# blairstar/NaturalDiffusion

Measured on AMD Instinct MI355X. Metric: images/sec at 15-step Natural Inference (CIFAR10 32x32, NCSN++), 3-stream throughput, higher is better.
Workload: dtype bf16; 1 GPU; CIFAR10 NI 15-step step_15_weight_173.npz B=512/GPU NCSN++ 61.8M bf16, ni_step fp64 history; nfe=15, batch_per_gpu=512, streams=3

## Files before the change

### include/natinf_ncsnpp.h

```cpp
#ifndef NATINF_NCSNPP_H
#define NATINF_NCSNPP_H

#include <stdint.h>
#include "natinf.h"

#ifdef __cplusplus
extern "C" {
#endif

typedef struct natinf_ncsnpp* natinf_ncsnpp_t;

#define NATINF_NCSNPP_KEEP_ACTIVATIONS 1
#define NATINF_NCSNPP_DDPM 2

int64_t natinf_ncsnpp_param_count(void);
int64_t natinf_ncsnpp_packed_bytes(void);
int64_t natinf_ncsnpp_handle_param_count(natinf_ncsnpp_t h);
int64_t natinf_ncsnpp_handle_packed_bytes(natinf_ncsnpp_t h);
int64_t natinf_ncsnpp_workspace_bytes(natinf_ncsnpp_t h, int max_batch);

int natinf_ncsnpp_create(natinf_ncsnpp_t* out, int flags);
int natinf_ncsnpp_destroy(natinf_ncsnpp_t h);

int natinf_ncsnpp_describe(natinf_ncsnpp_t h, char* buf, int cap);
// ... 22 lines not shown
int natinf_debug_conv_gn_fin(float* fin_scale, float* fin_shift, const float* gamma, const float* beta, int channels_per_group, float mul);
int natinf_debug_conv_gn(int res, int B, int N, int cin, int c1, const void* x, const float* scale, const float* shift, const void* w_packed, void* w_frag,
                         const void* a1, const float* bias_n, const void* resid, float out_scale, void* out, float* gn_part, int iters,
                         natinf_stream_t stream);
#define NATINF_ATTN_BLOCK_OFF_WQKV 0
#define NATINF_ATTN_BLOCK_OFF_W3 393216
#define NATINF_ATTN_BLOCK_OFF_FOLD_WQK 524288
#define NATINF_ATTN_BLOCK_OFF_FOLD_WVO 786432
#define NATINF_ATTN_BLOCK_OFF_FOLD_CQ 1048576
#define NATINF_ATTN_BLOCK_OFF_FOLD_BO 1049600
#define NATINF_ATTN_BLOCK_OFF_WQK_PACKED 1050624
#define NATINF_ATTN_BLOCK_OFF_WVO_PACKED 1181696
#define NATINF_ATTN_BLOCK_PACKED_BYTES 1312768
#define NATINF_ATTN_BLOCK_SCRATCH_BYTES_PER_SAMPLE 393216
int natinf_debug_attn_block(int plan, int B, const void* x, int x_ld, const float* scale, const float* shift, const float* w, const float* bias,
                            void* packed, void* scratch, void* out, int o_ld, float out_scale, float* gn_part, natinf_stream_t stream);
int natinf_set_gemm_variant(int variant);
int natinf_set_gemm_epilogue(int fp32_slab);
int natinf_set_gemm_pref512(int on);
int natinf_set_gemm_half_issue(int on);
int natinf_set_gemm_round_model(int on);
int natinf_set_gemm_w128(int on);
int natinf_set_gemm_raster(int rows);
int natinf_set_fuse_gn(int on);
int natinf_set_conv_gn_wide(int mask);
int natinf_set_conv_gn_w128(int mask);
int natinf_set_conv_gn_w128_min_k(int shape, int k);
int natinf_set_conv_gn_regw(int on);
int natinf_set_fuse_up(int on);
int natinf_set_fuse_up_fold(int on);
int natinf_debug_fold_up_weights(const float* w, int N, int cin, float w_mul, float* out_f32, void* out_packed, natinf_stream_t stream);
int natinf_debug_conv_up_fold(int B, int N, int cin, const void* x, const float* scale, const float* shift, const float* w, void* w_packed, void* h_scratch,
                              const float* bias_n, const float* rowvec, float out_scale, void* out, float* gn_part, int iters, natinf_stream_t stream);
int natinf_set_fuse_head(int on);
int natinf_set_fuse_gn8(int on);
int natinf_set_fuse_gn4(int on);
int natinf_set_fuse_fin(int on);
int natinf_set_conv_gn_warm(int mask);
int natinf_set_attn256(int on);
int natinf_set_attn_proj(int on);
int natinf_set_attn_waves8(int on);
int natinf_set_attn_block(int on);
int natinf_set_attn_qkv(int on);
int natinf_set_conv_gn8_tile(int one_image);
int natinf_set_gemm_splitk(int on);
int natinf_debug_set_splitk_workspace(float* ws, int max_slices);
int natinf_debug_timestamps(void* dev_buf16);

int natinf_ncsnpp_profile(natinf_ncsnpp_t h, int enable);
int natinf_ncsnpp_profile_read(natinf_ncsnpp_t h, double* ms_by_class , int64_t* launches_by_class );

int natinf_gemm_profile(int enable);
int natinf_gemm_profile_read(char* buf, int cap);

int natinf_ncsnpp_debug_tap(natinf_ncsnpp_t h, int module_idx, float* out, int64_t capacity_elems,
                            natinf_stream_t stream);

#ifdef __cplusplus
}
#endif
#endif
```

### naturaldiffusion_amd/_lib.py

```python
from __future__ import annotations

import ctypes as C
import os
from pathlib import Path

os.environ.setdefault("GPU_MAX_HW_QUEUES", "8")

_HERE = Path(__file__).resolve().parent
LIB_PATH = Path(os.environ.get("NATINF_LIB", _HERE / "libnatinf.so"))

if not LIB_PATH.exists():
    raise ImportError(
        f"{LIB_PATH} not found: build it with `make -C {_HERE / 'csrc'}` "
        "(or `python -c 'import __graft_entry__ as g; g.build()'`). "
        "naturaldiffusion_amd has no CPU or eager-PyTorch fallback.")

lib = C.CDLL(str(LIB_PATH))

_p, _i32, _i64, _f32, _f64 = C.c_void_p, C.c_int, C.c_int64, C.c_float, C.c_double

SIGNATURES = {
    "natinf_abi_version": (C.c_int, []),
    "natinf_strerror": (C.c_char_p, [_i32]),
    "natinf_probe": (C.c_int, []),
# ... 37 lines not shown
    "natinf_ncsnpp_param_count": (C.c_int64, []),
    "natinf_ncsnpp_workspace_bytes": (C.c_int64, [_p, _i32]),
    "natinf_ncsnpp_packed_bytes": (C.c_int64, []),
    "natinf_ncsnpp_handle_param_count": (_i64, [_p]),
    "natinf_ncsnpp_handle_packed_bytes": (_i64, [_p]),
    "natinf_ncsnpp_create": (C.c_int, [C.POINTER(_p), _i32]),
    "natinf_ncsnpp_describe": (C.c_int, [_p, C.c_char_p, _i32]),
    "natinf_ncsnpp_destroy": (C.c_int, [_p]),
    "natinf_ncsnpp_load": (C.c_int, [_p, _p, _i64, _p, _i64, _p]),
    "natinf_ncsnpp_share": (C.c_int, [_p, _p]),
    "natinf_ncsnpp_forward": (C.c_int, [_p, _p, _p, _p, _i32, _p, _i64, _p]),
    "natinf_ncsnpp_debug_tap": (C.c_int, [_p, _i32, _p, _i64, _p]),
    "natinf_ncsnpp_describe_gemms": (C.c_int, [_p, _i32, C.c_char_p, _i32]),
    "natinf_debug_gemm": (C.c_int, [_i32, _i32, _i32, _i32, _i32, _i32, _i32, _i32, _p, _p, _p, _p, _p, _i32, _f32, _i32, _p]),
    "natinf_set_gemm_variant": (C.c_int, [_i32]),
    "natinf_debug_timestamps": (C.c_int, [_p]),
    "natinf_set_gemm_epilogue": (C.c_int, [_i32]),
    "natinf_debug_gemm_fused": (C.c_int, [_i32, _i32, _i32, _i32, _p, _p, _p, _p, _p, _p, _i32, _p, _p, _f32, _i32, _p, _i32, _p, _p, _i32, _p]),
    "natinf_set_gemm_pref512": (C.c_int, [_i32]),
    "natinf_set_gemm_half_issue": (C.c_int, [_i32]),
    "natinf_set_gemm_raster": (C.c_int, [_i32]),
    "natinf_set_gemm_round_model": (C.c_int, [_i32]),
    "natinf_set_gemm_w128": (C.c_int, [_i32]),
    "natinf_set_fuse_gn": (C.c_int, [_i32]),
    "natinf_set_conv_gn_wide": (C.c_int, [_i32]),
    "natinf_set_attn_block": (C.c_int, [_i32]),
    "natinf_set_conv_gn_w128": (C.c_int, [_i32]),
    "natinf_set_conv_gn_w128_min_k": (C.c_int, [_i32, _i32]),
    "natinf_set_conv_gn_regw": (C.c_int, [_i32]),
    "natinf_set_fuse_up": (C.c_int, [_i32]),
    "natinf_set_fuse_up_fold": (C.c_int, [_i32]),
    "natinf_debug_fold_up_weights": (C.c_int, [_p, _i32, _i32, _f32, _p, _p, _p]),
    "natinf_debug_conv_up_fold": (C.c_int, [_i32, _i32, _i32, _p, _p, _p, _p, _p, _p, _p, _p, _f32, _p, _p, _i32, _p]),
    "natinf_set_fuse_head": (C.c_int, [_i32]),
    "natinf_set_fuse_gn8": (C.c_int, [_i32]),
    "natinf_set_fuse_gn4": (C.c_int, [_i32]),
    "natinf_set_fuse_fin": (C.c_int, [_i32]),
    "natinf_set_attn_proj": (C.c_int, [_i32]),
    "natinf_set_attn_waves8": (C.c_int, [_i32]),
    "natinf_set_attn_qkv": (C.c_int, [_i32]),
    "natinf_set_conv_gn_warm": (C.c_int, [_i32]),
    "natinf_set_attn256": (C.c_int, [_i32]),
    "natinf_set_conv_gn8_tile": (C.c_int, [_i32]),
    "natinf_set_gemm_splitk": (C.c_int, [_i32]),
    "natinf_debug_set_splitk_workspace": (C.c_int, [_p, _i32]),
    "natinf_debug_set_conv_operand": (C.c_int, [_i32, _p, _i32]),
    "natinf_debug_conv_gn": (C.c_int, [_i32, _i32, _i32, _i32, _i32, _p, _p, _p, _p, _p, _p, _p, _p, _f32, _p, _p, _i32, _p]),
    "natinf_debug_conv_gn_up": (C.c_int, [_i32]),
    "natinf_debug_conv_gn_fin": (C.c_int, [_p, _p, _p, _p, _i32, _f32]),
    "natinf_debug_attn_block": (C.c_int, [_i32, _i32, _p, _i32, _p, _p, _p, _p, _p, _p, _p, _i32, _f32, _p, _p]),
    "natinf_ncsnpp_profile": (C.c_int, [_p, _i32]),
    "natinf_ncsnpp_profile_read": (C.c_int, [_p, C.POINTER(C.c_double), C.POINTER(C.c_int64)]),
    "natinf_debug_quant_fp8_rows": (C.c_int, [_p, _p, _p, _i32, _i32, _p]),
    "natinf_debug_gemm_fp8": (C.c_int, [_i32, _i32, _i32, _p, _p, _p, _p, _p, _p, _p, _p, _i32, _i32, _p]),
    "natinf_dit_create": (C.c_int, [C.POINTER(_p), _i32, _i32, _i32, _i32]),
    "natinf_dit_create_sized": (C.c_int, [C.POINTER(_p), _i32, _i32, _i32, _i32, _i32]),
    "natinf_dit_input_size": (C.c_int, [_p]),
    "natinf_dit_attention_bf16": (C.c_int, [_p, _p, _p, _i32, _p, _i32, _i32, _i32, _i32, _i32, _i32, _p]),
    "natinf_dit_destroy": (C.c_int, [_p]),
    "natinf_dit_param_count": (C.c_int64, [_p]),
    "natinf_dit_packed_bytes": (C.c_int64, [_p]),
    "natinf_dit_workspace_bytes": (C.c_int64, [_p, _i32]),
    "natinf_dit_load": (C.c_int, [_p, _p, _i64, _p, _i64, _p]),
    "natinf_dit_forward": (C.c_int, [_p, _p, _p, _p, _p, _i32, _p, _i64, _p]),
    "natinf_dit_stream_sites": (C.c_int, [_p]),
    "natinf_dit_stream_status_reset": (C.c_int, [_p, _p, _p]),
# ... 132 lines not shown
```

### naturaldiffusion_amd/csrc/gemm_launch.h

```cpp
#pragma once
#include <hip/hip_runtime.h>
#include <stdint.h>
#include <stdio.h>
#include <string.h>
#include <string>
#include <type_traits>
#include <utility>
#include <vector>

#include "ncsnpp_kernels.h"
#include "gemm_dma.h"
#include "gemm_w128.h"
#include "conv_gn2.h"
#include "gemm_fp8.h"

using namespace ncsn;

bool configure_conv_ring();
namespace { bool configure_ncsnpp_kernels();
            bool configure_dit_attention();
            bool configure_flash_attention(); }
namespace ncsn_sg { bool configure(); bool has_tile(int variant); void launch_tile(const void* gemm_args, int variant, int raster, void* stream);
                    void launch_fp8(const void* gemm_args, int mxa, int w128, int raster, void* stream); void launch_splitk_reduce(const void* gemm_args, int slices, void* stream);
                    void launch_patch_embed(const float* z, const float* Wt, const float* bias, const float* pos, float* x, int C, int g, int D, int64_t rows, int x_f16, uint32_t* guard, void* stream); }
namespace ncsn_upf { bool configure(); void launch(const void* gemm_args, int epi, void* stream); void fold(const float* w, void* dst_bf16, float* dst_f32, int N, int Cin, float wmul, void* stream); }
namespace ncsn_cg3 { bool configure(); int tile_rows(int shape); int tile_cols(int shape); void launch(const void* gemm_args, int shape, int epi, void* stream); }

namespace {

int g_epi_fp32_slab = 0;
GemmArgs gemm_defaults() {
    GemmArgs g;
    memset(&g, 0, sizeof(g));
    g.epi_fp32_slab = g_epi_fp32_slab;
    g.taps = 1; g.batch = 1; g.scale = 1.0f; g.act = ACT_NONE; g.c_mode = OUT_BF16;
    return g;
}
constexpr int NUM_CU = 256;
enum GemmVariant {
    V_AUTO = 0, V_GENERIC = 1,
    V_DMA_256x256 = 2, V_DMA_256x128 = 3, V_DMA_128x128 = 4,
    V_RING_256x256 = 5, V_RING_256x128 = 6, V_RING_128x128 = 7,
    V_RING_64x128 = 8,
    V_RING_256x128_W4 = 9,
    V_DMA_256x128_W4 = 10,
    V_DMA_256x256_S = 11, V_DMA_128x128_S = 12,
    V_DMA_512x128 = 13,
    V_PATCH_256x256 = 14, V_PATCH_256x128 = 15,
    V_DMA_256x256_P = 16, V_DMA_256x128W4_P = 18,
    V_DMA_128x128_P = 17,
    V_8PH_256x256 = 19, V_8PH_NOPRIO = 20, V_8PH_READFIRST = 21, V_8PH_BOTH = 22,
    V_FP8_256x256 = 23,
    V_ABL_NODMA = 24, V_ABL_NOMFMA = 25,
    V_DMA_256x256_H = 26, V_DMA_512x128_H = 27,
    V_CONV_GN = 28,
    V_W128 = 29,
    V_W128_A = 30, V_W128_D = 31, V_W128_X = 32,
    V_COUNT
// ... 72 lines not shown
constexpr unsigned epi_mask(int v) { unsigned m = 1u; with_family(v, [&](auto f) { m = decltype(f)::EPI; }); return m; }
constexpr int variant_bm(int v) {
    int bm = (v == V_CONV_GN || v == V_FP8_256x256) ? 256 : 128;
    with_family(v, [&](auto f) { bm = decltype(f)::Cfg::BM_; });
    return bm;
}
static_assert(variant_bm(V_RING_64x128) == 64 && variant_bm(V_DMA_128x128_P) == 128 && variant_bm(V_RING_256x128_W4) == 256 && variant_bm(V_DMA_256x256_H) == 256 &&
              variant_bm(V_DMA_512x128_H) == 512 && variant_bm(V_W128) == 256 && variant_bm(V_GENERIC) == 128, "the block-tile rows choose_variant and the GroupNorm partial tables count on");
static_assert(variant_shipped(V_W128) && !variant_shipped(V_DMA_256x256) && !variant_shipped(V_W128_X) && epi_mask(V_GENERIC) == 1u, "retired ids stay refused");

constexpr unsigned EPI_CONV_GN = (1u << 1) | (1u << 2) | (1u << 5) | (1u << 6);
template <int RES_, bool WIDE, int TM = 8, int NG = 1, int TN = 4> struct CgShape {
    static constexpr int RES = RES_; using Cfg = ConvGn2Cfg<RES_, WIDE, TM, NG, TN>; static constexpr unsigned EPI = EPI_CONV_GN;
    template <int E> static constexpr auto kernel() { return &k_conv_gn2<RES_, WIDE, E, TM, NG, TN>; }
    static bool takes(int res, int bm) { return res == RES_ && (RES_ <= 8 || WIDE == (bm == 128)); }
};
using CgH4T = CgShape<4, true, 4, 2, 2>;
using ConvGnShapes = FamList<CgShape<32, false>, CgShape<32, true>, CgShape<16, false>, CgShape<16, true>, CgShape<8, true, 4>, CgH4T>;
template <class... S> void launch_conv_gn2(FamList<S...>, int res, int bm, int e, const GemmArgs& g, hipStream_t s) {
    ((S::takes(res, bm) && (launch_family<S>(e, g, s), true)) || ...);
}

constexpr int UPFOLD_W = 16, UPFOLD_BM = UPFOLD_W * UPFOLD_W, UPFOLD_BN = 256;

constexpr unsigned EPI_FP8 = 0xF;
template <bool MXA> struct FamF8     { using Cfg = CfgD256x256; static constexpr unsigned EPI = EPI_FP8; template <int E> static constexpr auto kernel() { return &k_gemm_fp8<MXA, E>; } };
template <bool MXA> struct FamF8W128 { using Cfg = W128F8Cfg;   static constexpr unsigned EPI = EPI_FP8; template <int E> static constexpr auto kernel() { return &k_gemm_w128_fp8<MXA, E>; } };
using Fp8Families = FamList<FamF8<false>, FamF8<true>, FamF8W128<false>, FamF8W128<true>>;

bool configure_gemm_kernels() {
    bool ok = hipFuncSetAttribute(reinterpret_cast<const void*>(&k_gemm_bf16), hipFuncAttributeMaxDynamicSharedMemorySize,
                                  GEMM_LDS_BYTES) == hipSuccess;
    ok = ok && set_lds<CfgR128x128>(&k_gemm_ring<2, 2, 4, 4, 4, 9>) && set_lds<W128Cfg>(&k_gemm_w128<9>) &&
         configure_families(GemmFamilies{}) && configure_families(ConvGnShapes{}) && ncsn_upf::configure() && configure_families(Fp8Families{}) &&
         ncsn_cg3::configure() && ncsn_sg::configure() && ::configure_conv_ring() && configure_ncsnpp_kernels() && configure_dit_attention() && configure_flash_attention();
    if (!ok) (void)hipGetLastError();
    return ok;
}


int packed_epi(const GemmArgs& g, int bm);
int g_cg3 = 7;
int g_cg_wide = 3;
int g_cg3_min_k[3] = {2304, 0, 2304};
inline int conv_gn3_shape(const GemmArgs& g) {
    const int res = 1 << g.logW;
    if (!g_cg3 || !g.b_frag || g.N % 128) return -1;
    int sh = -1;
    if (res == 32) sh = g.N % 256 ? ((g_cg3 & 1) ? 0 : -1) : ((g_cg3 & 2) ? 1 : -1);
    else if (res == 16) sh = (g.N % 256 == 0 && (g_cg3 & 4)) ? 2 : -1;
    if (sh >= 0 && 9 * g.a0_C + (g.a1 ? g.a1_C : 0) < g_cg3_min_k[sh]) sh = -1;
    return sh;
}
inline int conv_gn_bm(const GemmArgs& g) {
    const int res = 1 << g.logW;
    if (const int sh3 = conv_gn3_shape(g); sh3 >= 0) return ncsn_cg3::tile_rows(sh3);
    if (res == 8 || res == 4) return 64;
    if (res == 32) return ((g_cg_wide & 2) && g.N % 256 == 0 && g.b_frag) ? 128 : 256;
    return ((g_cg_wide & 1) && res == 16 && g.N % 256 == 0) ? 128 : 256;
}
inline int conv_gn_part_rows(const GemmArgs& g) { const int res = 1 << g.logW; return res <= 8 ? res * res : conv_gn_bm(g); }
inline bool conv_gn_regw(const GemmArgs& g) { return g.b_frag && (conv_gn3_shape(g) >= 0 || g.N % ((conv_gn_bm(g) <= 128 && (1 << g.logW) != 4) ? 256 : 128) == 0); }
inline int conv_gn_epi(const GemmArgs& g) { GemmArgs t = g; t.epi_fp32_slab = 0; return packed_epi(t, conv_gn_part_rows(g)); }
inline bool conv_gn_ok(const GemmArgs& g) {
    if (!g.gn_scale || !g.gn_shift || !g.gn_folded || g.taps != 9 || g.batch != 1 || g.a0_C % BK || (g.a1 && g.a1_C % BK)) return false;
    const int res = 1 << g.logW;
    if (g.logHW != 2 * g.logW || (res != 32 && res != 16 && res != 8 && res != 4) || g.N % 8) return false;
// ... 225 lines not shown
```

### naturaldiffusion_amd/csrc/ncsnpp.hip

```cpp
#include <hip/hip_runtime.h>
#include <stdint.h>
#include <stdio.h>
#include <string.h>
#include <stdlib.h>
#include <functional>
#include <map>
#include <memory>
#include <string>
#include <vector>

#include "natinf_ncsnpp.h"
#include "gemm_launch.h"
#include "engine_core.h"
#include "head_conv.h"
#include "attn256.h"
#include "attn_qkv.h"
#include "attn_blk256.h"

namespace {

constexpr int NF = 128, IMG = 32, TEMB = 512, NLEVEL = 4;
constexpr int CH_MULT[NLEVEL] = {1, 2, 2, 2};
constexpr float GN_EPS = 1e-6f;
constexpr float INV_SQRT2 = 0.70710678118654752440f;
inline bool attn_at(int res) { return res == 16; }

enum Kind { K_LIN, K_CONV, K_RES, K_ATTN, K_GN, K_DOWN, K_UP };
const char* kind_name(int k) { static const char* n[] = {"lin", "conv", "res", "attn", "gn", "down", "up"}; return n[k]; }

struct Mod { int idx, kind, cin, cout, up, down, res; int64_t poff; };

enum { CLS_GEMM = 0, CLS_OTHER = 1, CLS_CONV_GN = 2, CLS_CONV_GN8 = 3, N_CLS = 4 };

int g_fuse_head = 1;
constexpr int ATTN_BLK_DEFAULT = 2;
int g_attn_blk = ATTN_BLK_DEFAULT;
int g_attn_qkv = 1;
int g_attn_w8 = 1;
int g_attn_proj = 1;
int g_fuse_gn8 = 1;
int g_fuse_fin = 3;
int g_fuse_gn4 = 1;
int g_fuse_gn = 1;
constexpr int UP_FOLD_DEFAULT = 1;
int g_fuse_up_fold = UP_FOLD_DEFAULT;
int g_fuse_up = 1;

}

struct natinf_ncsnpp : EngineCore {
    int flags = 0;
    std::vector<Mod> mods;
    std::vector<int> op_cls;
    bool prof = false;
    struct Rec { hipEvent_t a, b; int cls; };
    std::vector<Rec> recs;
    std::vector<hipEvent_t> pool;
    std::map<int, TRef> taps;
    uint64_t plan_sig = 0;
    int last_B = 0; unsigned char* last_ws = nullptr;
    std::vector<unsigned char> fin_done;
};

namespace {

bool configure_ncsnpp_kernels() {
    return hipFuncSetAttribute(reinterpret_cast<const void*>(&k_head_conv), hipFuncAttributeMaxDynamicSharedMemorySize, HeadConvCfg::LDS_BYTES) == hipSuccess &&
           hipFuncSetAttribute(reinterpret_cast<const void*>(&k_qkv256), hipFuncAttributeMaxDynamicSharedMemorySize, QKV_LDS_BYTES) == hipSuccess &&
           hipFuncSetAttribute(reinterpret_cast<const void*>(&k_attn256<false>), hipFuncAttributeMaxDynamicSharedMemorySize, A256_LDS_BYTES) == hipSuccess &&
           hipFuncSetAttribute(reinterpret_cast<const void*>(&k_attn256<true>), hipFuncAttributeMaxDynamicSharedMemorySize, A256_LDS_BYTES) == hipSuccess &&
           hipFuncSetAttribute(reinterpret_cast<const void*>(&k_attn256<true, 8>), hipFuncAttributeMaxDynamicSharedMemorySize, A256_LDS_BYTES) == hipSuccess &&
           hipFuncSetAttribute(reinterpret_cast<const void*>(&k_attn_blk256), hipFuncAttributeMaxDynamicSharedMemorySize, ABLK_LDS_BYTES) == hipSuccess &&
           hipFuncSetAttribute(reinterpret_cast<const void*>(&k_attn_blk256_v2), hipFuncAttributeMaxDynamicSharedMemorySize, ABLK2_LDS_BYTES) == hipSuccess;
}

struct AttnBlk256 {
    int plan = 0;
    int B = 0;
// ... 8 lines not shown
void pack_attn_qkv_w(const float* w0, const float* w1, const float* w2, bf16* wqkvf, hipStream_t s) {
    hipLaunchKernelGGL(k_pack_qkv_w, dim3(3 * 256), dim3(256), 0, s, w0, w1, w2, wqkvf);
}
void pack_attn_w3(const float* w3, bf16* w3f, hipStream_t s) { hipLaunchKernelGGL(k_pack_attn_w3, dim3(256), dim3(256), 0, s, w3, w3f); }
void pack_attn_fold(const float* w0, const float* w1, const float* w2, const float* w3, const float* b0, const float* b2, const float* b3,
                    float* fq, float* cq, float* fv, float* bo, bf16* wqf2, bf16* wvof2, hipStream_t s) {
    hipLaunchKernelGGL(k_attn_fold_w, dim3(257), dim3(256), 0, s, w0, w1, w2, w3, b0, b2, b3, fq, cq, fv, bo);
    hipLaunchKernelGGL(k_pack_qkv_w, dim3(256), dim3(256), 0, s, (const float*)fq, (const float*)fq, (const float*)fq, wqf2, 1);
    hipLaunchKernelGGL(k_pack_attn_w3, dim3(256), dim3(256), 0, s, (const float*)fv, wvof2);
}
void launch_attn_qkv256(const AttnBlk256& a, hipStream_t s) {
    hipLaunchKernelGGL(k_qkv256, dim3((unsigned)a.B), dim3(512), QKV_LDS_BYTES, s, a.x, a.x_ld, a.sc, a.sh, a.wqkvf, a.bqk, a.bv, a.qk, a.vT);
}
int launch_attn_blk256(const AttnBlk256& a, hipStream_t s) {
    constexpr int C = 256;
    if (a.plan == 2) {
        hipLaunchKernelGGL(k_attn_blk256_v2, dim3((unsigned)a.B), dim3(512), ABLK2_LDS_BYTES, s, a.x, a.x_ld, a.sc, a.sh,
                           a.wqf2, a.cq2, 1.0f / sqrtf((float)C), a.wvof2, a.bo2, a.out, a.o_ld, a.out_scale, a.gn_part, a.gn_quads);
        return 256;
    }
    if (a.plan == 1) {
        hipLaunchKernelGGL(k_attn_blk256, dim3((unsigned)a.B), dim3(512), ABLK_LDS_BYTES, s, a.x, a.x_ld, a.sc, a.sh,
                           a.wqkvf, a.bqk, a.bv, a.qk, a.vT, 1.0f / sqrtf((float)C), a.w3f, a.b3, a.out, a.o_ld, a.out_scale, a.gn_part, a.gn_quads);
        return 256;
    }
    if (g_attn_w8) {
        hipLaunchKernelGGL((k_attn256<true, 8>), dim3((unsigned)a.B), dim3(512), A256_LDS_BYTES, s, (const bf16*)a.qk, 2 * C, C, (const bf16*)a.vT, a.out, a.o_ld,
                           1.0f / sqrtf((float)C), a.w3f, a.b3, a.x, a.x_ld, a.out_scale, a.gn_part, a.gn_quads);
        return 256;
    }
    hipLaunchKernelGGL(k_attn256<true>, dim3((unsigned)(2 * a.B)), dim3(256), A256_LDS_BYTES, s, (const bf16*)a.qk, 2 * C, C, (const bf16*)a.vT, a.out, a.o_ld,
                       1.0f / sqrtf((float)C), a.w3f, a.b3, a.x, a.x_ld, a.out_scale, a.gn_part, a.gn_quads);
    return 128;
}

struct Builder : PlanBuilder {
    natinf_ncsnpp& E;
    int dense_total = 0; int64_t dense_w = 0, dense_b = 0, dense_out = 0;

    const bool ddpm;
    const int NUM_RES;
    const float res_scale;
    explicit Builder(natinf_ncsnpp& e) : PlanBuilder(e), E(e), ddpm((e.flags & NATINF_NCSNPP_DDPM) != 0), NUM_RES(ddpm ? 2 : 4), res_scale(ddpm ? 1.0f : INV_SQRT2) {
        arena.keep = (e.flags & NATINF_NCSNPP_KEEP_ACTIVATIONS) != 0;
    }

    void op(int cls, OpFn f) { E.ops.push_back(std::move(f)); E.op_cls.push_back(cls); }

    void pack_conv(int64_t src, int64_t dst, int N, int Cin, int taps, int dst_ld, int koff, int tapstride, float wmul = 1.0f) {
        const int chunked = taps == 9 && Cin % BK == 0;
        E.packs.push_back([=](const PackCtx& p) {
            const int64_t n = (int64_t)N * Cin * taps;
            hipLaunchKernelGGL(k_pack_conv, dim3(grid1d(n, 256, 1 << 30)), dim3(256), 0, p.stream, p.params + src,
                               reinterpret_cast<bf16*>(p.packed + dst), N, Cin, taps, dst_ld, koff, tapstride, chunked, wmul);
        });
    }
    void pack_frag(int64_t src_packed, int64_t dst, int N, int ld, int cin, int c1) {
        E.packs.push_back([=](const PackCtx& p) {
            const int64_t n = (int64_t)(N / 16) * (9 * (cin / 32) + c1 / 32) * 64;
            hipLaunchKernelGGL(k_pack_frag, dim3(grid1d(n, 256, 1 << 30)), dim3(256), 0, p.stream, reinterpret_cast<const bf16*>(p.packed + src_packed),
                               reinterpret_cast<bf16*>(p.packed + dst), N, ld, cin, c1);
        });
    }
    void pack_fold_up(int64_t src, int64_t dst, int N, int Cin, float wmul) {
        E.packs.push_back([=](const PackCtx& p) {
            ncsn_upf::fold(p.params + src, p.packed + dst, nullptr, N, Cin, wmul, (void*)p.stream);
// ... 500 lines not shown
            const Mod& m0 = M[mi++]; const Mod& m1 = M[mi++]; (void)m0; (void)m1;
            const int64_t pw0 = take((int64_t)TEMB * NF), pb0 = take(TEMB), pw1 = take((int64_t)TEMB * TEMB), pb1 = take(TEMB);
            const int64_t w0 = wres((int64_t)TEMB * NF * 2), w1 = wres((int64_t)TEMB * TEMB * 2);
            pack_conv(pw0, w0, TEMB, NF, 1, NF, 0, NF); pack_conv(pw1, w1, TEMB, TEMB, 1, TEMB, 0, TEMB);
            const int64_t b0 = pack_f32(pb0, TEMB), b1 = pack_f32(pb1, TEMB);
            const int64_t dw = dense_w, db = dense_b, dout = dense_out; const int dtot = dense_total;
            op(CLS_OTHER, [=](const Ctx& c) {
                hipLaunchKernelGGL(k_time_embed, dim3(grid1d((int64_t)c.B * 128)), dim3(256), 0, c.stream, c.labels, c.at<bf16>(emb), c.B);
            });
            op(CLS_GEMM, [=](const Ctx& c) {
                GemmArgs g = gemm_defaults();
                g.a0 = c.at<bf16>(emb); g.a0_ld = NF; g.a0_C = NF; g.M = c.B; g.N = TEMB;
                g.b = c.w<bf16>(w0); g.b_ld = NF; g.bias_n = c.w<float>(b0); g.act = ACT_SILU;
                g.c = c.at<bf16>(t1); g.c_ld = TEMB;
                launch_gemm(g, c.stream);
                g = gemm_defaults();
                g.a0 = c.at<bf16>(t1); g.a0_ld = TEMB; g.a0_C = TEMB; g.M = c.B; g.N = TEMB;
                g.b = c.w<bf16>(w1); g.b_ld = TEMB; g.bias_n = c.w<float>(b1); g.act = ACT_SILU;
                g.c = c.at<bf16>(t2); g.c_ld = TEMB;
                launch_gemm(g, c.stream);
                g = gemm_defaults();
                g.a0 = c.at<bf16>(t2); g.a0_ld = TEMB; g.a0_C = TEMB; g.M = c.B; g.N = dtot;
                g.b = c.w<bf16>(dw); g.b_ld = TEMB; g.bias_n = c.w<float>(db);
                g.c = c.at<float>(dout); g.c_ld = dtot; g.c_mode = OUT_F32;
                launch_gemm(g, c.stream);
            });
        }
        int si = 0;
        TRef cur = skip_slot(si++);
        {
            const Mod& m = M[mi++];
            const int64_t pw = take((int64_t)NF * 27), pb = take(NF);
            const int64_t w = wres((int64_t)NF * 64 * 2);
            pack_zero(w, (int64_t)NF * 64);
            pack_conv(pw, w, NF, 3, 9, 64, 0, 3);
            const int64_t b = pack_f32(pb, NF);
            const int64_t a0 = arena.alloc((int64_t)IMG * IMG * 64 * 2);
            const TRef dst = cur;
            const Part po = register_output(dst);
            op(CLS_OTHER, [=](const Ctx& c) {
                const int64_t rows = (int64_t)c.B * IMG * IMG;
                hipLaunchKernelGGL(k_stem_im2col, dim3((unsigned)((rows * 8 + 255) / 256)), dim3(256), 0, c.stream, c.x, c.at<bf16>(a0), rows);
            });
            op(CLS_GEMM, [=](const Ctx& c) {
                const int64_t rows = (int64_t)c.B * IMG * IMG;
                GemmArgs g = gemm_defaults();
                g.a0 = c.at<bf16>(a0); g.a0_ld = 64; g.a0_C = 64; g.M = (int)rows; g.N = NF;
                g.b = c.w<bf16>(w); g.b_ld = 64; g.bias_n = c.w<float>(b);
                g.c = c.act(dst); g.c_ld = dst.ld;
                if (po.valid) { g.gn_part = c.at<float>(po.off); g.gn_quads = po.quads; }
                const int bm = launch_gemm(g, c.stream);
                if (po.valid) c.part_bm[po.id] = bm;
            });
            arena.release(a0);
            E.taps[m.idx] = dst;
        }
        int res = IMG;
        for (int l = 0; l < NLEVEL; ++l) {
            for (int b = 0; b < NUM_RES; ++b) {
                const Mod& m = M[mi++];
                const TRef dst = skip_slot(si++);
                if (attn_at(res)) {
                    TRef tmp = new_act(res, m.cout);
                    emit_res(m, cur, tmp);
                    emit_attn(M[mi++], tmp, dst);
                    arena.release(tmp.off);
                } else {
                    emit_res(m, cur, dst);
                }
                cur = dst;
            }
            if (l != NLEVEL - 1) {
                const Mod& m = M[mi++];
                const TRef dst = skip_slot(si++);
                if (ddpm) emit_downconv(m, cur, dst); else emit_res(m, cur, dst);
                cur = dst; res /= 2;
            }
        }
        {
            TRef a = new_act(res, cur.C), b = new_act(res, cur.C);
            emit_res(M[mi++], cur, a);
            emit_attn(M[mi++], a, b);
            arena.release(a.off);
            emit_res(M[mi++], b, h_slot(0));
// ... 96 lines not shown
const natinf_ncsnpp& reference_engine() {
    static natinf_ncsnpp* e = [] {
        int* knobs[] = {&g_fuse_gn, &g_fuse_up, &g_fuse_head, &g_fuse_gn8, &g_fuse_gn4, &g_fuse_fin, &g_attn_qkv, &g_attn_proj};
        int saved[sizeof(knobs) / sizeof(knobs[0])];
        for (size_t i = 0; i < sizeof(knobs) / sizeof(knobs[0]); ++i) { saved[i] = *knobs[i]; *knobs[i] = 1; }
        g_fuse_fin = 3;
        const int saved_fold = g_fuse_up_fold;
        g_fuse_up_fold = 0;
        natinf_ncsnpp* r = make_engine(0);
        g_fuse_up_fold = saved_fold;
        for (size_t i = 0; i < sizeof(knobs) / sizeof(knobs[0]); ++i) *knobs[i] = saved[i];
        return r;
    }();
    return *e;
}

}

extern "C" {

int64_t natinf_ncsnpp_param_count(void) { return reference_engine().n_params; }
int64_t natinf_ncsnpp_packed_bytes(void) { return reference_engine().packed_bytes; }

int64_t natinf_ncsnpp_handle_param_count(natinf_ncsnpp_t h) { return h ? h->n_params : NATINF_EINVAL; }
int64_t natinf_ncsnpp_handle_packed_bytes(natinf_ncsnpp_t h) { return h ? h->packed_bytes : NATINF_EINVAL; }

int64_t natinf_ncsnpp_workspace_bytes(natinf_ncsnpp_t h, int max_batch) {
    if (!h || max_batch <= 0) return NATINF_EINVAL;
    return h->ws_per_image * (int64_t)max_batch;
}

static uint64_t plan_signature() {
    const int k[] = {g_fuse_head, g_attn_qkv, g_attn_w8, g_attn_proj, g_fuse_gn8, g_fuse_fin, g_fuse_gn4, g_fuse_gn, g_cg_wide, g_fuse_up,
                     g_attn_blk , g_fuse_up_fold, g_cg3 };
    uint64_t h = 1469598103934665603ull;
    for (int v : k) h = (h ^ (uint64_t)(v & 0xff)) * 1099511628211ull;
    return h;
}

int natinf_ncsnpp_create(natinf_ncsnpp_t* out, int flags) {
    if (!out || (flags & ~(NATINF_NCSNPP_KEEP_ACTIVATIONS | NATINF_NCSNPP_DDPM))) return NATINF_EINVAL;
    natinf_ncsnpp* e = make_engine(flags);
    if (!e) return NATINF_ESTATE;
    e->plan_sig = plan_signature();
    *out = e;
    return NATINF_OK;
}

int natinf_ncsnpp_destroy(natinf_ncsnpp_t h) {
    if (!h) return NATINF_EINVAL;
    for (auto& r : h->recs) { (void)hipEventDestroy(r.a); (void)hipEventDestroy(r.b); }
    for (auto e : h->pool) (void)hipEventDestroy(e);
    delete h;
    return NATINF_OK;
}

int natinf_ncsnpp_describe(natinf_ncsnpp_t h, char* buf, int cap) {
    if (!h || !buf || cap <= 0) return NATINF_EINVAL;
    std::string s;
    char line[160];
    for (const auto& m : h->mods) {
        snprintf(line, sizeof(line), "%d %s %d %d %d %d %d %lld\n", m.idx, kind_name(m.kind), m.cin, m.cout, m.up, m.down, m.res,
                 (long long)m.poff);
        s += line;
    }
    if ((int)s.size() + 1 > cap) return NATINF_EINVAL;
    memcpy(buf, s.c_str(), s.size() + 1);
// ... 171 lines not shown
        hipLaunchKernelGGL(k_pack_frag, dim3(grid1d(n, 256, 1 << 30)), dim3(256), 0, (hipStream_t)stream, (const bf16*)w_packed, (bf16*)w_frag, N, g.b_ld, cin, c1);
    }
    for (int i = 0; i < iters; ++i) launch_gemm(g, (hipStream_t)stream);
    return hipGetLastError() == hipSuccess ? NATINF_OK : NATINF_ELAUNCH;
}

int natinf_debug_fold_up_weights(const float* w, int N, int cin, float w_mul, float* out_f32, void* out_packed, natinf_stream_t stream) {
    if (!w || N <= 0 || cin <= 0 || (!out_f32 && !out_packed) || (out_packed && cin % 64)) return NATINF_EINVAL;
    ncsn_upf::fold(w, out_packed, out_f32, N, cin, w_mul, stream);
    return hipGetLastError() == hipSuccess ? NATINF_OK : NATINF_ELAUNCH;
}
int natinf_debug_conv_up_fold(int B, int N, int cin, const void* x, const float* scale, const float* shift, const float* w, void* w_packed, void* h_scratch,
                              const float* bias_n, const float* rowvec, float out_scale, void* out, float* gn_part, int iters, natinf_stream_t stream) {
    if (B <= 0 || N != UPFOLD_BN || cin <= 0 || cin % 64 || !x || !scale || !shift || !w || !w_packed || !h_scratch || !out || iters <= 0) return NATINF_EINVAL;
    static bool configured = false;
    if (!configured) { if (!configure_gemm_kernels()) return NATINF_ENODEV; configured = true; }
    hipStream_t s = (hipStream_t)stream;
    constexpr int W = UPFOLD_W, logW = 4;
    ncsn_upf::fold(w, w_packed, nullptr, N, cin, 1.0f, stream);
    hipLaunchKernelGGL(k_gn_apply, dim3((unsigned)((W + 2 + GN_ROWS - 1) / GN_ROWS), (unsigned)B), dim3(256), 0, s, (const bf16*)x, cin, cin, logW, 2 * logW, scale, shift,
                       (bf16*)h_scratch, (bf16*)nullptr, ACT_SILU, RS_NONE, 1);
    GemmArgs g = gemm_defaults();
    g.a0 = (const bf16*)h_scratch; g.a0_ld = cin; g.a0_padded = 1; g.a0_C = cin; g.taps = 4; g.logW = logW; g.logHW = 2 * logW;
    g.M = B * W * W; g.N = 4 * N; g.b = (const bf16*)w_packed; g.b_ld = 4 * cin; g.bias_n = bias_n;
    g.rowvec = rowvec; g.rowvec_ld = N; g.log_rows_per_sample = 2 * logW; g.scale = out_scale;
    g.c = out; g.c_ld = N; g.gn_part = gn_part; g.gn_quads = N / 4;
    if (!up_fold_epi(g)) return NATINF_EINVAL;
    g_launch_error = 0;
    for (int i = 0; i < iters; ++i) launch_gemm(g, s);
    if (g_launch_error) { g_launch_error = 0; return NATINF_EINVAL; }
    return hipGetLastError() == hipSuccess ? NATINF_OK : NATINF_ELAUNCH;
}

int natinf_debug_attn_block(int plan, int B, const void* x, int x_ld, const float* scale, const float* shift, const float* w, const float* bias,
                            void* packed, void* scratch, void* out, int o_ld, float out_scale, float* gn_part, natinf_stream_t stream) {
    if (plan < 0 || plan > 2 || B < 1 || !x || !scale || !shift || !w || !bias || !packed || !out || x_ld < 256 || x_ld % 8 || o_ld < 256 || o_ld % 8 ||
        (plan != 2 && !scratch)) return NATINF_EINVAL;
    static bool configured = false;
    if (!configured) { if (!configure_gemm_kernels()) return NATINF_ENODEV; configured = true; }
    constexpr int64_t WW = 256 * 256;
    unsigned char* pk = reinterpret_cast<unsigned char*>(packed);
    hipStream_t s = (hipStream_t)stream;
    AttnBlk256 a;
    a.plan = plan; a.B = B; a.x = (const bf16*)x; a.x_ld = x_ld; a.sc = scale; a.sh = shift;
    a.out = (bf16*)out; a.o_ld = o_ld; a.out_scale = out_scale; a.gn_part = reinterpret_cast<float2*>(gn_part); a.gn_quads = 64;
    if (plan == 2) {
        float* fq = reinterpret_cast<float*>(pk + NATINF_ATTN_BLOCK_OFF_FOLD_WQK); float* fv = reinterpret_cast<float*>(pk + NATINF_ATTN_BLOCK_OFF_FOLD_WVO);
        float* cq = reinterpret_cast<float*>(pk + NATINF_ATTN_BLOCK_OFF_FOLD_CQ); float* bo = reinterpret_cast<float*>(pk + NATINF_ATTN_BLOCK_OFF_FOLD_BO);
        bf16* wqf2 = reinterpret_cast<bf16*>(pk + NATINF_ATTN_BLOCK_OFF_WQK_PACKED); bf16* wvof2 = reinterpret_cast<bf16*>(pk + NATINF_ATTN_BLOCK_OFF_WVO_PACKED);
        pack_attn_fold(w, w + WW, w + 2 * WW, w + 3 * WW, bias, bias + 512, bias + 768, fq, cq, fv, bo, wqf2, wvof2, s);
        a.wqf2 = wqf2; a.cq2 = cq; a.wvof2 = wvof2; a.bo2 = bo;
    } else {
        bf16* wqkvf = reinterpret_cast<bf16*>(pk + NATINF_ATTN_BLOCK_OFF_WQKV); bf16* w3f = reinterpret_cast<bf16*>(pk + NATINF_ATTN_BLOCK_OFF_W3);
        pack_attn_qkv_w(w, w + WW, w + 2 * WW, wqkvf, s);
        pack_attn_w3(w + 3 * WW, w3f, s);
        a.wqkvf = wqkvf; a.bqk = bias; a.bv = bias + 512; a.w3f = w3f; a.b3 = bias + 768;
        a.qk = reinterpret_cast<bf16*>(scratch); a.vT = a.qk + (int64_t)B * 256 * 512;
        if (plan == 0) launch_attn_qkv256(a, s);
    }
    launch_attn_blk256(a, s);
    return hipGetLastError() == hipSuccess ? NATINF_OK : NATINF_ELAUNCH;
}

int natinf_debug_quant_fp8_rows(const float* w, void* q, float* row_scale, int rows, int cols, natinf_stream_t stream) {
    if (!w || !q || !row_scale || rows <= 0 || cols <= 0 || cols % 2) return NATINF_EINVAL;
    hipLaunchKernelGGL(k_pack_fp8_rows, dim3((unsigned)((rows + 3) / 4)), dim3(256), 0, (hipStream_t)stream, w, (uint8_t*)q, row_scale, rows, cols);
// ... 19 lines not shown
int natinf_debug_timestamps(void* dev_buf16) {
#ifdef NATINF_DEV
    g_dbg_ts = reinterpret_cast<unsigned long long*>(dev_buf16); return NATINF_OK;
#else
    (void)dev_buf16; return NATINF_ESTATE;
#endif
}

int natinf_set_gemm_raster(int rows) { g_raster_g = rows; return NATINF_OK; }
int natinf_set_fuse_gn(int on) { g_fuse_gn = on != 0; return NATINF_OK; }
int natinf_set_fuse_gn8(int on) { g_fuse_gn8 = on != 0; return NATINF_OK; }
int natinf_set_attn256(int on) { return on ? NATINF_OK : NATINF_ESTATE; }
int natinf_set_conv_gn_warm(int mask) { if (mask < 0 || mask > 15) return NATINF_EINVAL; g_cg_warm = mask; return NATINF_OK; }
int natinf_set_attn_block(int on) { g_attn_blk = on < 0 ? ATTN_BLK_DEFAULT : (on > 2 ? 2 : on); return NATINF_OK; }
int natinf_set_attn_qkv(int on) { g_attn_qkv = on != 0; return NATINF_OK; }
int natinf_set_attn_waves8(int on) { g_attn_w8 = on != 0; return NATINF_OK; }
int natinf_set_attn_proj(int on) { g_attn_proj = on != 0; return NATINF_OK; }
int natinf_set_fuse_fin(int on) {
    if (on < 0 || on > 3) return NATINF_EINVAL;
    static const int mask[4] = {0, 3, 1, 2};
    g_fuse_fin = mask[on];
    return NATINF_OK;
}
int natinf_set_gemm_round_model(int on) { g_round_model = on != 0; g_round_model_w128 = on >= 10 ? on : 13; return NATINF_OK; }
int natinf_set_gemm_w128(int on) { g_w128 = on < 0 ? 0 : (on > 2 ? 2 : on); return NATINF_OK; }
int natinf_set_fuse_gn4(int on) { g_fuse_gn4 = on != 0; return NATINF_OK; }
int natinf_set_conv_gn8_tile(int one_image) { return one_image ? NATINF_OK : NATINF_ESTATE; }
int natinf_set_fuse_head(int on) { g_fuse_head = on != 0; return NATINF_OK; }
int natinf_set_conv_gn_w128(int mask) { if (mask < 0 || mask > 7) return NATINF_EINVAL; g_cg3 = mask; return NATINF_OK; }
int natinf_set_conv_gn_w128_min_k(int shape, int k) { if (shape < 0 || shape > 2 || k < 0) return NATINF_EINVAL; g_cg3_min_k[shape] = k; return NATINF_OK; }
int natinf_set_conv_gn_wide(int mask) { if (mask < 0 || mask > 3) return NATINF_EINVAL; g_cg_wide = mask; return NATINF_OK; }
int natinf_set_conv_gn_regw(int on) { return on ? NATINF_OK : NATINF_ESTATE; }
int natinf_set_fuse_up(int on) { g_fuse_up = on != 0; return NATINF_OK; }
int natinf_set_fuse_up_fold(int on) { g_fuse_up_fold = on < 0 ? UP_FOLD_DEFAULT : on != 0; return NATINF_OK; }
int natinf_set_gemm_splitk(int on) { g_splitk = on != 0; return NATINF_OK; }
int natinf_debug_set_splitk_workspace(float* ws, int max_slices) { g_dbg_splitk_ws = ws; g_dbg_splitk_max = ws ? max_slices : 0; return NATINF_OK; }
int natinf_set_gemm_half_issue(int on) { return on ? NATINF_OK : NATINF_ESTATE; }
int natinf_set_gemm_pref512(int on) { g_pref_512 = on != 0; return NATINF_OK; }
int natinf_set_gemm_epilogue(int fp32_slab) { g_epi_fp32_slab = fp32_slab != 0; return NATINF_OK; }

int natinf_set_gemm_variant(int variant) {
    if (variant < 0 || variant >= V_COUNT) return NATINF_EINVAL;
    if (!variant_shipped(variant) || variant == V_CONV_GN || variant == V_FP8_256x256) return NATINF_ESTATE;
    g_force_variant = variant;
    return NATINF_OK;
}

int natinf_gemm_profile(int enable) { g_gemm_prof.on = enable != 0; return NATINF_OK; }
int natinf_gemm_profile_read(char* buf, int cap) {
    if (!buf || cap <= 0) return NATINF_EINVAL;
    std::map<std::string, std::pair<double, int64_t>> by;
    std::vector<std::string> order;
    int rc = NATINF_OK;
    for (auto& e : g_gemm_prof.ev) {
        float ms = 0.f;
        if (hipEventSynchronize(e.b) != hipSuccess || hipEventElapsedTime(&ms, e.a, e.b) != hipSuccess) { (void)hipGetLastError(); rc = NATINF_ELAUNCH; }
        else {
            auto it = by.find(e.tag);
            if (it == by.end()) { order.push_back(e.tag); it = by.emplace(e.tag, std::make_pair(0.0, (int64_t)0)).first; }
            it->second.first += ms; it->second.second += 1;
        }
        g_gemm_prof.pool.emplace_back(e.a, e.b);
    }
    g_gemm_prof.ev.clear();
    if (rc != NATINF_OK) return rc;
    std::string out;
// ... 50 lines not shown
```

Baseline: 3569 images/s.

## Fuse stem im2col into a direct 3x3 stem conv kernel

```diff
diff --git a/include/natinf_ncsnpp.h b/include/natinf_ncsnpp.h
--- a/include/natinf_ncsnpp.h
+++ b/include/natinf_ncsnpp.h
@@ -78,6 +78,9 @@
 int natinf_debug_fold_up_weights(const float* w, int N, int cin, float w_mul, float* out_f32, void* out_packed, natinf_stream_t stream);
 int natinf_debug_conv_up_fold(int B, int N, int cin, const void* x, const float* scale, const float* shift, const float* w, void* w_packed, void* h_scratch,
                               const float* bias_n, const float* rowvec, float out_scale, void* out, float* gn_part, int iters, natinf_stream_t stream);
+int natinf_set_stem_direct(int on);
+int natinf_debug_stem_conv(int direct, int B, const float* x, const float* w, const float* bias, void* w_packed, void* a_scratch, void* out, int out_ld, float* gn_part,
+                           int* bm_out, natinf_stream_t stream);
 int natinf_set_fuse_head(int on);
 int natinf_set_fuse_gn8(int on);
 int natinf_set_fuse_gn4(int on);
diff --git a/naturaldiffusion_amd/_lib.py b/naturaldiffusion_amd/_lib.py
--- a/naturaldiffusion_amd/_lib.py
+++ b/naturaldiffusion_amd/_lib.py
@@ -93,6 +93,8 @@
     "natinf_set_fuse_up_fold": (C.c_int, [_i32]),
     "natinf_debug_fold_up_weights": (C.c_int, [_p, _i32, _i32, _f32, _p, _p, _p]),
     "natinf_debug_conv_up_fold": (C.c_int, [_i32, _i32, _i32, _p, _p, _p, _p, _p, _p, _p, _p, _f32, _p, _p, _i32, _p]),
+    "natinf_set_stem_direct": (C.c_int, [_i32]),
+    "natinf_debug_stem_conv": (C.c_int, [_i32, _i32, _p, _p, _p, _p, _p, _p, _i32, _p, C.POINTER(_i32), _p]),
     "natinf_set_fuse_head": (C.c_int, [_i32]),
     "natinf_set_fuse_gn8": (C.c_int, [_i32]),
     "natinf_set_fuse_gn4": (C.c_int, [_i32]),
diff --git a/naturaldiffusion_amd/csrc/gemm_launch.h b/naturaldiffusion_amd/csrc/gemm_launch.h
--- a/naturaldiffusion_amd/csrc/gemm_launch.h
+++ b/naturaldiffusion_amd/csrc/gemm_launch.h
@@ -24,6 +24,8 @@
                     void launch_fp8(const void* gemm_args, int mxa, int w128, int raster, void* stream); void launch_splitk_reduce(const void* gemm_args, int slices, void* stream);
                     void launch_patch_embed(const float* z, const float* Wt, const float* bias, const float* pos, float* x, int C, int g, int D, int64_t rows, int x_f16, uint32_t* guard, void* stream); }
 namespace ncsn_upf { bool configure(); void launch(const void* gemm_args, int epi, void* stream); void fold(const float* w, void* dst_bf16, float* dst_f32, int N, int Cin, float wmul, void* stream); }
+namespace ncsn_stem { bool configure(); void launch(const float* x, const void* w32, const void* gemm_args, void* stream); }
+constexpr int STEM_BM = 256, STEM_KP = 32;
 namespace ncsn_cg3 { bool configure(); int tile_rows(int shape); int tile_cols(int shape); void launch(const void* gemm_args, int shape, int epi, void* stream); }
 
 namespace {
@@ -162,7 +164,7 @@
     bool ok = hipFuncSetAttribute(reinterpret_cast<const void*>(&k_gemm_bf16), hipFuncAttributeMaxDynamicSharedMemorySize,
                                   GEMM_LDS_BYTES) == hipSuccess;
     ok = ok && set_lds<CfgR128x128>(&k_gemm_ring<2, 2, 4, 4, 4, 9>) && set_lds<W128Cfg>(&k_gemm_w128<9>) &&
-         configure_families(GemmFamilies{}) && configure_families(ConvGnShapes{}) && ncsn_upf::configure() && configure_families(Fp8Families{}) &&
+         configure_families(GemmFamilies{}) && configure_families(ConvGnShapes{}) && ncsn_upf::configure() && ncsn_stem::configure() && configure_families(Fp8Families{}) &&
          ncsn_cg3::configure() && ncsn_sg::configure() && ::configure_conv_ring() && configure_ncsnpp_kernels() && configure_dit_attention() && configure_flash_attention();
     if (!ok) (void)hipGetLastError();
     return ok;
diff --git a/naturaldiffusion_amd/csrc/ncsnpp.hip b/naturaldiffusion_amd/csrc/ncsnpp.hip
--- a/naturaldiffusion_amd/csrc/ncsnpp.hip
+++ b/naturaldiffusion_amd/csrc/ncsnpp.hip
@@ -44,6 +44,7 @@
 int g_fuse_gn = 1;
 constexpr int UP_FOLD_DEFAULT = 1;
 int g_fuse_up_fold = UP_FOLD_DEFAULT;
+int g_stem_direct = 1;
 int g_fuse_up = 1;
 
 }
@@ -118,6 +119,41 @@
     hipLaunchKernelGGL(k_attn256<true>, dim3((unsigned)(2 * a.B)), dim3(256), A256_LDS_BYTES, s, (const bf16*)a.qk, 2 * C, C, (const bf16*)a.vT, a.out, a.o_ld,
                        1.0f / sqrtf((float)C), a.w3f, a.b3, a.x, a.x_ld, a.out_scale, a.gn_part, a.gn_quads);
     return 128;
+}
+
+struct StemConv {
+    int direct = 0;
+    int B = 0;
+    const float* x = nullptr;
+    const bf16* w = nullptr;
+    bf16* a0 = nullptr;
+    const float* bias = nullptr;
+    bf16* out = nullptr; int o_ld = 0;
+    float* gn_part = nullptr; int gn_quads = 0;
+};
+void pack_stem_w(const float* w, bf16* dst, int direct, hipStream_t s) {
+    hipLaunchKernelGGL(k_fill_bf16_zero, dim3((NF * 64 + 255) / 256), dim3(256), 0, s, dst, (int64_t)NF * 64);
+    hipLaunchKernelGGL(k_pack_conv, dim3((NF * 27 + 255) / 256), dim3(256), 0, s, w, dst, NF, 3, 9, direct ? STEM_KP : 64, 0, 3, 0, 1.0f);
+}
+void launch_stem_im2col(const StemConv& t, hipStream_t s) {
+    const int64_t rows = (int64_t)t.B * IMG * IMG;
+    hipLaunchKernelGGL(k_stem_im2col, dim3((unsigned)((rows * 8 + 255) / 256)), dim3(256), 0, s, t.x, t.a0, rows);
+}
+int launch_stem(const StemConv& t, hipStream_t s) {
+    const int64_t rows = (int64_t)t.B * IMG * IMG;
+    GemmArgs g = gemm_defaults();
+    g.a0 = t.a0; g.a0_ld = 64; g.a0_C = 64; g.M = (int)rows; g.N = NF;
+    g.b = t.w; g.b_ld = 64; g.bias_n = t.bias;
+    g.c = t.out; g.c_ld = t.o_ld;
+    g.gn_part = t.gn_part; g.gn_quads = t.gn_quads;
+    if (g_record || !t.direct) return launch_gemm(g, s);
+    if (!t.gn_part || t.o_ld % 8) { g_launch_error = 1; return STEM_BM; }
+    GemmProf::Rec r;
+    const bool prof = g_gemm_prof.on && g_gemm_prof.begin(r, s);
+    if (prof) r.tag = gemm_row((int)rows, NF, STEM_KP, 0, 9, 1, "stem_conv", 2);
+    ncsn_stem::launch(t.x, t.w, &g, (void*)s);
+    if (prof) g_gemm_prof.end(r, s);
+    return STEM_BM;
 }
 
 struct Builder : PlanBuilder {
@@ -684,24 +720,22 @@
             const Mod& m = M[mi++];
             const int64_t pw = take((int64_t)NF * 27), pb = take(NF);
             const int64_t w = wres((int64_t)NF * 64 * 2);
-            pack_zero(w, (int64_t)NF * 64);
-            pack_conv(pw, w, NF, 3, 9, 64, 0, 3);
+            const TRef dst = cur;
+            const Part po = register_output(dst);
+            const int direct = g_stem_direct && po.valid;
+            E.packs.push_back([=](const PackCtx& p) { pack_stem_w(p.params + pw, reinterpret_cast<bf16*>(p.packed + w), direct, p.stream); });
             const int64_t b = pack_f32(pb, NF);
             const int64_t a0 = arena.alloc((int64_t)IMG * IMG * 64 * 2);
-            const TRef dst = cur;
-            const Part po = register_output(dst);
-            op(CLS_OTHER, [=](const Ctx& c) {
-                const int64_t rows = (int64_t)c.B * IMG * IMG;
-                hipLaunchKernelGGL(k_stem_im2col, dim3((unsigned)((rows * 8 + 255) / 256)), dim3(256), 0, c.stream, c.x, c.at<bf16>(a0), rows);
-            });
+            auto stem = [=](const Ctx& c) {
+                StemConv t;
+                t.direct = direct; t.B = c.B; t.x = c.x; t.w = c.w<bf16>(w); t.a0 = c.at<bf16>(a0); t.bias = c.w<float>(b);
+                t.out = c.act(dst); t.o_ld = dst.ld;
+                if (po.valid) { t.gn_part = c.at<float>(po.off); t.gn_quads = po.quads; }
+                return t;
+            };
+            if (!direct) op(CLS_OTHER, [=](const Ctx& c) { launch_stem_im2col(stem(c), c.stream); });
             op(CLS_GEMM, [=](const Ctx& c) {
-                const int64_t rows = (int64_t)c.B * IMG * IMG;
-                GemmArgs g = gemm_defaults();
-                g.a0 = c.at<bf16>(a0); g.a0_ld = 64; g.a0_C = 64; g.M = (int)rows; g.N = NF;
-                g.b = c.w<bf16>(w); g.b_ld = 64; g.bias_n = c.w<float>(b);
-                g.c = c.act(dst); g.c_ld = dst.ld;
-                if (po.valid) { g.gn_part = c.at<float>(po.off); g.gn_quads = po.quads; }
-                const int bm = launch_gemm(g, c.stream);
+                const int bm = launch_stem(stem(c), c.stream);
                 if (po.valid) c.part_bm[po.id] = bm;
             });
             arena.release(a0);
@@ -864,7 +898,7 @@
 
 static uint64_t plan_signature() {
     const int k[] = {g_fuse_head, g_attn_qkv, g_attn_w8, g_attn_proj, g_fuse_gn8, g_fuse_fin, g_fuse_gn4, g_fuse_gn, g_cg_wide, g_fuse_up,
-                     g_attn_blk , g_fuse_up_fold, g_cg3 };
+                     g_attn_blk , g_fuse_up_fold, g_stem_direct , g_cg3 };
     uint64_t h = 1469598103934665603ull;
     for (int v : k) h = (h ^ (uint64_t)(v & 0xff)) * 1099511628211ull;
     return h;
@@ -1102,6 +1136,24 @@
     return hipGetLastError() == hipSuccess ? NATINF_OK : NATINF_ELAUNCH;
 }
 
+int natinf_debug_stem_conv(int direct, int B, const float* x, const float* w, const float* bias, void* w_packed, void* a_scratch, void* out, int out_ld, float* gn_part,
+                           int* bm_out, natinf_stream_t stream) {
+    if (B <= 0 || (int64_t)B * IMG * IMG >= (1LL << 31) || !x || !w || !w_packed || !out || out_ld < NF || out_ld % 8 || !gn_part || (!direct && !a_scratch)) return NATINF_EINVAL;
+    static bool configured = false;
+    if (!configured) { if (!configure_gemm_kernels()) return NATINF_ENODEV; configured = true; }
+    hipStream_t s = (hipStream_t)stream;
+    StemConv t;
+    t.direct = direct != 0; t.B = B; t.x = x; t.w = (const bf16*)w_packed; t.a0 = (bf16*)a_scratch; t.bias = bias; t.out = (bf16*)out; t.o_ld = out_ld;
+    t.gn_part = gn_part; t.gn_quads = NF / 4;
+    pack_stem_w(w, (bf16*)w_packed, t.direct, s);
+    g_launch_error = 0;
+    if (!t.direct) launch_stem_im2col(t, s);
+    const int bm = launch_stem(t, s);
+    if (bm_out) *bm_out = bm;
+    if (g_launch_error) { g_launch_error = 0; return NATINF_EINVAL; }
+    return hipGetLastError() == hipSuccess ? NATINF_OK : NATINF_ELAUNCH;
+}
+
 int natinf_debug_attn_block(int plan, int B, const void* x, int x_ld, const float* scale, const float* shift, const float* w, const float* bias,
                             void* packed, void* scratch, void* out, int o_ld, float out_scale, float* gn_part, natinf_stream_t stream) {
     if (plan < 0 || plan > 2 || B < 1 || !x || !scale || !shift || !w || !bias || !packed || !out || x_ld < 256 || x_ld % 8 || o_ld < 256 || o_ld % 8 ||
@@ -1187,6 +1239,7 @@
 int natinf_set_conv_gn_wide(int mask) { if (mask < 0 || mask > 3) return NATINF_EINVAL; g_cg_wide = mask; return NATINF_OK; }
 int natinf_set_conv_gn_regw(int on) { return on ? NATINF_OK : NATINF_ESTATE; }
 int natinf_set_fuse_up(int on) { g_fuse_up = on != 0; return NATINF_OK; }
+int natinf_set_stem_direct(int on) { g_stem_direct = on < 0 ? 1 : on != 0; return NATINF_OK; }
 int natinf_set_fuse_up_fold(int on) { g_fuse_up_fold = on < 0 ? UP_FOLD_DEFAULT : on != 0; return NATINF_OK; }
 int natinf_set_gemm_splitk(int on) { g_splitk = on != 0; return NATINF_OK; }
 int natinf_debug_set_splitk_workspace(float* ws, int max_slices) { g_dbg_splitk_ws = ws; g_dbg_splitk_max = ws ? max_slices : 0; return NATINF_OK; }
diff --git a/naturaldiffusion_amd/csrc/stem_conv.h b/naturaldiffusion_amd/csrc/stem_conv.h
--- /dev/null
+++ b/naturaldiffusion_amd/csrc/stem_conv.h
@@ -0,0 +1,73 @@
+#pragma once
+#include "gemm_dma.h"
+
+namespace ncsn {
+
+struct StemCfg {
+    static constexpr int WM = 2, WN = 2, TM = 8, TN = 4, THREADS = WM * WN * 64;
+    static constexpr int BM_ = WM * TM * 16, BN_ = WN * TN * 16, KP = 32;
+    static constexpr int IMG_W = 32, ROWS = BM_ / IMG_W, PH = ROWS + 2, PW = IMG_W + 2, CIN = 3;
+    using Epi = RingCfg<WM, WN, TM, TN, 3>::Epi;
+    static constexpr int A_BYTES = BM_ * KP * 2;
+    static constexpr int PATCH_BYTES = (CIN * PH * PW * 2 + 15) / 16 * 16;
+    static constexpr int LDS_BYTES = Epi::PACK_BYTES > A_BYTES + PATCH_BYTES ? Epi::PACK_BYTES : A_BYTES + PATCH_BYTES;
+    static_assert(BM_ % IMG_W == 0 && (IMG_W * IMG_W) % BM_ == 0 && Epi::PACK_OK, "whole image rows per tile, whole tiles per image");
+};
+
+__global__ __launch_bounds__(StemCfg::THREADS, 2) void k_stem_conv(const float* __restrict__ x, const bf16* __restrict__ w32, const GemmArgs g)
+{
+    using Cfg = StemCfg;
+    constexpr int TM = Cfg::TM, TN = Cfg::TN, PH = Cfg::PH, PW = Cfg::PW, W = Cfg::IMG_W;
+    extern __shared__ __attribute__((aligned(16))) unsigned char smem[];
+    lds_poison();
+    const int tid = threadIdx.x, lane = tid & 63;
+    const int wave = __builtin_amdgcn_readfirstlane(tid >> 6);
+    const int wm = wave / Cfg::WN, wn = wave % Cfg::WN;
+    const int m0 = blockIdx.x * Cfg::BM_;
+    const int b = m0 / (W * W), y0 = (m0 % (W * W)) / W;
+    const int frow = lane & 15, fq = lane >> 4;
+
+    bf16x8 fb[TN];
+#pragma unroll
+    for (int j = 0; j < TN; ++j) fb[j] = __builtin_bit_cast(bf16x8, gload_u4(w32 + (wn * TN * 16 + j * 16 + frow) * Cfg::KP + fq * 8));
+
+    bf16* patch = reinterpret_cast<bf16*>(smem + Cfg::A_BYTES);
+    const float* xb = x + (int64_t)b * (Cfg::CIN * W * W);
+    for (int e = tid; e < Cfg::CIN * PH * PW; e += Cfg::THREADS) {
+        const int c = e / (PH * PW), r = e - c * (PH * PW), yy = r / PW, xx = r - yy * PW;
+        const int sy = y0 - 1 + yy, sx = xx - 1;
+        float v = 0.f;
+        if ((unsigned)sy < (unsigned)W && (unsigned)sx < (unsigned)W) v = xb[(c * W + sy) * W + sx];
+        patch[e] = (bf16)v;
+    }
+    __syncthreads();
+    {
+        const int py = tid / W, px = tid % W;
+        bf16x8 ch[Cfg::KP / 8];
+#pragma unroll
+        for (int k = 0; k < Cfg::KP; ++k) {
+            const int tap = k / 3, c = k - tap * 3;
+            ch[k >> 3][k & 7] = k < 9 * Cfg::CIN ? patch[(c * PH + py + tap / 3) * PW + px + tap % 3] : (bf16)0.0f;
+        }
+        const int sw = (0x1320 >> (((tid >> 2) & 3) * 4)) & 3;
+#pragma unroll
+        for (int q = 0; q < Cfg::KP / 8; ++q) *reinterpret_cast<bf16x8*>(smem + tid * (Cfg::KP * 2) + ((q ^ sw) << 4)) = ch[q];
+    }
+    __syncthreads();
+    bf16x8 fa[TM];
+    {
+        const int sw = (0x1320 >> (((frow >> 2) & 3) * 4)) & 3;
+#pragma unroll
+        for (int i = 0; i < TM; ++i) fa[i] = *reinterpret_cast<const bf16x8*>(smem + (wm * TM * 16 + i * 16 + frow) * (Cfg::KP * 2) + ((fq ^ sw) << 4));
+    }
+    __syncthreads();
+    f32x4 acc[TM][TN];
+#pragma unroll
+    for (int i = 0; i < TM; ++i)
+#pragma unroll
+        for (int j = 0; j < TN; ++j)
+            acc[i][j] = __builtin_amdgcn_mfma_f32_16x16x32_bf16(fb[j], fa[i], f32x4{0.f, 0.f, 0.f, 0.f}, 0, 0, 0);
+    tile_epilogue<Cfg::WM, Cfg::WN, TM, TN, Cfg::Epi, 2>(g, smem, acc, m0, 0, 0, tid, lane, wm, wn);
+}
+
+}
diff --git a/naturaldiffusion_amd/csrc/stem_conv.hip b/naturaldiffusion_amd/csrc/stem_conv.hip
--- /dev/null
+++ b/naturaldiffusion_amd/csrc/stem_conv.hip
@@ -0,0 +1,21 @@
+#include <hip/hip_runtime.h>
+#include <stdint.h>
+#include <string.h>
+
+namespace {
+#include "stem_conv.h"
+}
+using namespace ncsn;
+
+namespace ncsn_stem {
+static_assert(StemCfg::BM_ == 256 && StemCfg::KP == 32, "gemm_launch.h: STEM_BM, STEM_KP");
+__attribute__((visibility("hidden"))) bool configure() {
+    return hipFuncSetAttribute(reinterpret_cast<const void*>(&k_stem_conv), hipFuncAttributeMaxDynamicSharedMemorySize, StemCfg::LDS_BYTES) == hipSuccess;
+}
+__attribute__((visibility("hidden"))) void launch(const float* x, const void* w32, const void* gemm_args, void* stream) {
+    GemmArgs g;
+    memcpy(&g, gemm_args, sizeof(g));
+    hipLaunchKernelGGL(k_stem_conv, dim3((unsigned)(g.M / StemCfg::BM_)), dim3(StemCfg::THREADS), StemCfg::LDS_BYTES, reinterpret_cast<hipStream_t>(stream), x,
+                       reinterpret_cast<const bf16*>(w32), g);
+}
+}
```

Result: no change. 3576 images/s, median of 6 (+0.2%).
